# facebookresearch/vggsfm

Measured on NVIDIA H100. Metric: BA iterations/sec, higher is better.
Workload: dtype f64

## Files before the change

vggsfm_b200/csrc/chol.cu:

```cuda
#include <stdlib.h>
#include <algorithm>
#include <map>
#include <vector>
#include <tuple>
#include "common.cuh"

namespace vgg {

constexpr int CB = 128;
constexpr int CLD = 132;
constexpr int C_RPC = 16;
constexpr int C_RPC_MAX = 32;
constexpr int CT = 64;
constexpr int C_THREADS = 256;

__device__ __forceinline__ double fast_rsqrt(double p) {
  double r;
  asm("rsqrt.approx.ftz.f64 %0, %1;" : "=d"(r) : "d"(p));
  const double hp = 0.5 * p;
  r = r * fma(-hp * r, r, 1.5);
  r = r * fma(-hp * r, r, 1.5);
  return r;
}
constexpr double CHOL_PMIN = 2.2250738585072014e-308;

template <bool PROBE>
__device__ __forceinline__ int cta_chol128(double* Ls, double* dinv, int* fail_sm, int tid, int xr,
                                           long long* prof = nullptr) {
  const int lane = tid & 31, warp = tid >> 5;
  __shared__ __align__(16) double Lh[64];
  if (tid == 0) *fail_sm = 0;
  __syncthreads();
  auto tri_row = [](int e) { return (e >= 1) + (e >= 3) + (e >= 6) + (e >= 10) + (e >= 15) + (e >= 21) + (e >= 28); };
  const int pi0 = tri_row(lane), pj0 = lane - pi0 * (pi0 + 1) / 2;
  const int e1 = lane < 4 ? lane + 32 : 35;
  const int pi1 = tri_row(e1), pj1 = e1 - pi1 * (pi1 + 1) / 2;
  long long pacc[6] = {0, 0, 0, 0, 0, 0}, plast = 0;
  const bool ptid = PROBE && (tid == 0 || tid == 32);
  if (ptid) plast = clock64();
#define CHOL_MARK(ph)                         \
  if (ptid) {                                 \
    const long long t_ = clock64();           \
    pacc[ph] += t_ - plast;                   \
    plast = t_;                               \
  }
  auto leaf = [&](int c0) {
    double a[8];
    const int r = c0 + (lane & 7);
#pragma unroll
    for (int c = 0; c < 8; c += 2) {
      const double2 v = *reinterpret_cast<const double2*>(Ls + r * CLD + c0 + c);
      a[c] = v.x;
      a[c + 1] = v.y;
    }
    int fail = 0;
    double mydinv = 1.0;
#pragma unroll
    for (int j = 0; j < 8; j += 2) {
      const double A = __shfl_sync(0xffffffffu, a[j], j);
      const double B = __shfl_sync(0xffffffffu, a[j], j + 1);
      const double C = __shfl_sync(0xffffffffu, a[j + 1], j + 1);
      const double AC = A * C;
      const double det = fma(-B, B, AC);
      double ia = fast_rsqrt(A);
      double ib = (A * ia) * fast_rsqrt(det);
      double l10 = B * ia;
      const bool good = A >= CHOL_PMIN && det >= CHOL_PMIN && AC < 1e280 && AC > 1e-280;
      if (!good) {
        if (!(A >= CHOL_PMIN)) {
          if (fail == 0) fail = c0 + j + 1;
          ia = 1.0;
          l10 = B;
        }
        const double p1 = fma(-l10, l10, C);
        if (!(p1 >= CHOL_PMIN)) {
          if (fail == 0) fail = c0 + j + 2;
          ib = 1.0;
        } else {
          ib = rsqrt(p1);
        }
      }
      const double x0 = a[j] * ia;
      const double x1 = fma(-x0, l10, a[j + 1]) * ib;
      a[j] = x0;
      a[j + 1] = x1;
      if (lane == j) {
        dinv[c0 + j] = ia;
        dinv[c0 + j + 1] = ib;
        mydinv = ia;
      }
      if (lane == j + 1) mydinv = ib;
#pragma unroll
      for (int c = j + 2; c < 8; ++c) {
        const double l0 = __shfl_sync(0xffffffffu, x0, c);
        const double l1 = __shfl_sync(0xffffffffu, x1, c);
        if (lane >= c) a[c] = fma(-x1, l1, fma(-x0, l0, a[c]));
      }
    }
    if (lane < 8) {
#pragma unroll
      for (int c = 0; c < 8; ++c) Ls[r * CLD + c0 + c] = (c <= lane) ? a[c] : 0.0;
#pragma unroll
      for (int c = 0; c < 8; ++c) Lh[lane * 8 + c] = (c < lane) ? a[c] * mydinv : 0.0;
    }
    if (lane == 0 && fail && *fail_sm == 0) *fail_sm = fail;
  };
  auto row_update = [&](int r, int c0, int jb, int js, int jend) {
    double li[8];
#pragma unroll
    for (int k = 0; k < 8; k += 2) {
      const double2 v = *reinterpret_cast<const double2*>(Ls + r * CLD + c0 + k);
      li[k] = v.x;
      li[k + 1] = v.y;
    }
    int j = jb;
    for (; j + js <= jend; j += 2 * js) {
      const double* l0 = Ls + j * CLD + c0;
      const double* l1 = Ls + (j + js) * CLD + c0;
      double s0 = Ls[r * CLD + j], s1 = Ls[r * CLD + j + js];
#pragma unroll
      for (int k = 0; k < 8; k += 2) {
        const double2 u = *reinterpret_cast<const double2*>(l0 + k);
        const double2 w = *reinterpret_cast<const double2*>(l1 + k);
        s0 = fma(-li[k], u.x, s0);
        s1 = fma(-li[k], w.x, s1);
        s0 = fma(-li[k + 1], u.y, s0);
        s1 = fma(-li[k + 1], w.y, s1);
      }
      Ls[r * CLD + j] = s0;
      Ls[r * CLD + j + js] = s1;
    }
    if (j <= jend) {
      const double* l0 = Ls + j * CLD + c0;
      double s0 = Ls[r * CLD + j];
#pragma unroll
      for (int k = 0; k < 8; k += 2) {
        const double2 u = *reinterpret_cast<const double2*>(l0 + k);
        s0 = fma(-li[k], u.x, s0);
        s0 = fma(-li[k + 1], u.y, s0);
      }
      Ls[r * CLD + j] = s0;
    }
  };
  if (warp == 0) leaf(0);
  __syncthreads();
  CHOL_MARK(0)
  for (int sp = 0; sp < CB / 32; ++sp) {
    const int c32 = sp * 32;
    for (int mp = 0; mp < 4; ++mp) {
      const int c0 = c32 + mp * 8;
      {
        const int r = c0 + 8 + tid;
        if (r < CB + xr) {
          double x[8];
#pragma unroll
          for (int c = 0; c < 8; c += 2) {
            const double2 v = *reinterpret_cast<const double2*>(Ls + r * CLD + c0 + c);
            x[c] = v.x;
            x[c + 1] = v.y;
          }
#pragma unroll
          for (int m = 0; m < 8; ++m) x[m] *= dinv[c0 + m];
#pragma unroll
          for (int m = 1; m < 8; ++m) {
#pragma unroll
            for (int k = 0; k < m; ++k) x[m] = fma(-x[k], Lh[m * 8 + k], x[m]);
          }
#pragma unroll
          for (int c = 0; c < 8; c += 2) *reinterpret_cast<double2*>(Ls + r * CLD + c0 + c) = make_double2(x[c], x[c + 1]);
        }
      }
      __syncthreads();
      CHOL_MARK(1)
      if (mp < 3) {
        const int n0 = c0 + 8;
        if (warp == 0) {
          {
            const double* ri = Ls + (n0 + pi0) * CLD + c0;
            const double* rj = Ls + (n0 + pj0) * CLD + c0;
            const double* ri1 = Ls + (n0 + pi1) * CLD + c0;
            const double* rj1 = Ls + (n0 + pj1) * CLD + c0;
            double s0 = Ls[(n0 + pi0) * CLD + n0 + pj0], s1 = 0.0;
            double u0 = Ls[(n0 + pi1) * CLD + n0 + pj1], u1 = 0.0;
#pragma unroll
            for (int k = 0; k < 8; k += 4) {
              const double2 a0 = *reinterpret_cast<const double2*>(ri + k), a1 = *reinterpret_cast<const double2*>(ri + k + 2);
              const double2 b0 = *reinterpret_cast<const double2*>(rj + k), b1 = *reinterpret_cast<const double2*>(rj + k + 2);
              const double2 c0v = *reinterpret_cast<const double2*>(ri1 + k), c1v = *reinterpret_cast<const double2*>(ri1 + k + 2);
              const double2 d0 = *reinterpret_cast<const double2*>(rj1 + k), d1 = *reinterpret_cast<const double2*>(rj1 + k + 2);
              s0 = fma(-a0.x, b0.x, s0);
              s1 = fma(-a0.y, b0.y, s1);
              u0 = fma(-c0v.x, d0.x, u0);
              u1 = fma(-c0v.y, d0.y, u1);
              s0 = fma(-a1.x, b1.x, s0);
              s1 = fma(-a1.y, b1.y, s1);
              u0 = fma(-c1v.x, d1.x, u0);
              u1 = fma(-c1v.y, d1.y, u1);
            }
            Ls[(n0 + pi0) * CLD + n0 + pj0] = s0 + s1;
            if (lane < 4) Ls[(n0 + pi1) * CLD + n0 + pj1] = u0 + u1;
          }
          __syncwarp();
          leaf(n0);
        } else {
          const int t = tid - 32;
          for (int rr = t >> 1; n0 + rr < CB + xr; rr += 112) {
            const int r = n0 + rr, half = t & 1;
            const int jend = min(r, c32 + 31);
            if (r < n0 + 8) continue;
            row_update(r, c0, n0 + half, 2, jend);
          }
        }
        CHOL_MARK(2)
        __syncthreads();
        CHOL_MARK(3)
      }
    }
    const int t0 = c32 + 32;
    const int nrb = (CB - t0) / 32;
    if (nrb > 0) {
      const int ntile = nrb * (nrb + 1);
      const int nxt = xr ? (CB - t0) / 16 : 0;
      const int rend = CB + xr;
      const int g = lane >> 2, q = lane & 3;
      bool leaf_pending = warp == 0;
      for (int t = warp == 0 ? 0 : warp; t < ntile + nxt; t += (warp == 0 ? ntile + nxt : C_THREADS / 32 - 1)) {
        int R0, C0, nrow16 = 2;
        if (t < ntile) {
          int rb = 0, cb = t;
          while (cb >= 2 * rb + 2) { cb -= 2 * rb + 2; ++rb; }
          R0 = t0 + rb * 32;
          C0 = t0 + cb * 16;
        } else {
          R0 = CB;
          C0 = t0 + (t - ntile) * 16;
          nrow16 = (xr + 15) / 16;
        }
        double c[2][2][4];
#pragma unroll
        for (int i = 0; i < 2; ++i)
#pragma unroll
          for (int j = 0; j < 2; ++j) c[i][j][0] = c[i][j][1] = c[i][j][2] = c[i][j][3] = 0.0;
#pragma unroll
        for (int kk = c32; kk < c32 + 32; kk += 16) {
          double a[2][8], b[2][4];
#pragma unroll
          for (int j = 0; j < 2; ++j)
#pragma unroll
            for (int e = 0; e < 4; ++e) b[j][e] = Ls[(C0 + j * 8 + g) * CLD + kk + q + 4 * e];
#pragma unroll
          for (int i = 0; i < 2; ++i) {
            if (i < nrow16) {
#pragma unroll
              for (int e = 0; e < 8; ++e) {
                const int r = R0 + i * 16 + g + 8 * (e & 1);
                a[i][e] = r < rend ? Ls[r * CLD + kk + q + 4 * (e >> 1)] : 0.0;
              }
#pragma unroll
              for (int j = 0; j < 2; ++j) dmma_m16n8k16(c[i][j], a[i], b[j]);
            }
          }
        }
#pragma unroll
        for (int i = 0; i < 2; ++i) {
          if (i >= nrow16) continue;
#pragma unroll
          for (int h = 0; h < 2; ++h) {
            const int r = R0 + i * 16 + g + 8 * h;
            if (r >= rend) continue;
#pragma unroll
            for (int j = 0; j < 2; ++j) {
              const int col = C0 + j * 8 + 2 * q;
              if (col > r) continue;
              double* pp = Ls + r * CLD + col;
              if (col + 1 <= r) {
                double2 v = *reinterpret_cast<double2*>(pp);
                v.x -= c[i][j][2 * h];
                v.y -= c[i][j][2 * h + 1];
                *reinterpret_cast<double2*>(pp) = v;
              } else {
                *pp -= c[i][j][2 * h];
              }
            }
          }
        }
        if (leaf_pending) {
          __syncwarp();
          leaf(t0);
          leaf_pending = false;
        }
      }
      CHOL_MARK(4)
      __syncthreads();
      CHOL_MARK(5)
    }
  }
#undef CHOL_MARK
  if (ptid) {
#pragma unroll
    for (int i = 0; i < 6; ++i) prof[(tid == 32 ? 6 : 0) + i] = pacc[i];
  }
  return *fail_sm;
}

__global__ void __launch_bounds__(C_THREADS, 1) chol128_probe_kernel(const double* __restrict__ A, double* __restrict__ L,
                                                                      long long* __restrict__ prof, int reps, int xr) {
  extern __shared__ __align__(16) double cp_smem[];
  __shared__ double dinv[CB];
  __shared__ int fail_sm;
  const int tid = threadIdx.x;
  long long total = 0;
  for (int rep = 0; rep < reps; ++rep) {
    for (int e = tid; e < CB * CB; e += C_THREADS) cp_smem[(e >> 7) * CLD + (e & 127)] = A[e];
    for (int e = tid; e < xr * CB; e += C_THREADS)
      cp_smem[(CB + (e >> 7)) * CLD + (e & 127)] = A[(CB - xr + (e >> 7)) * CB + (e & 127)];
    __syncthreads();
    const long long t0 = clock64();
    cta_chol128<true>(cp_smem, dinv, &fail_sm, tid, xr, prof);
    __syncthreads();
    total = clock64() - t0;
  }
  if (tid == 0) prof[12] = total;
  for (int e = tid; e < CB * CB; e += C_THREADS) L[e] = ((e & 127) <= (e >> 7)) ? cp_smem[(e >> 7) * CLD + (e & 127)] : 0.0;
}

constexpr int CHOL_SPIN_LIMIT = 1 << 22;
constexpr int CHOL_INFO_STALLED = 0x7fffffff;

__global__ void __launch_bounds__(C_THREADS, 1) chol_panel_kernel(int n, int lda, int k0, double* __restrict__ A,
                                                                   double* __restrict__ Ldiag ,
                                                                   int* __restrict__ info, int* __restrict__ flags,
                                                                   int fuse, int band_end, int arrow_lo, int xr) {
  extern __shared__ __align__(16) double cp_smem[];
  double* Ls = cp_smem;
  double* Ts = cp_smem + CB * CLD;
  __shared__ double dinv[CB];
  __shared__ int fail_sm;
  const int tid = threadIdx.x, lane = tid & 31, warp = tid >> 5;
  const int nb = min(CB, n - k0);
  const bool solver = blockIdx.x > 0;
  const int band_hi = min(band_end, n);
  const int chunks1r = (max(0, band_hi - (k0 + CB)) + xr - 1) / xr;
  const int cidx = (int)blockIdx.x - 1;
  const int r0 = cidx < chunks1r ? k0 + CB + cidx * xr : arrow_lo + (cidx - chunks1r) * xr;
  const int nrows = solver ? min(xr, (cidx < chunks1r ? band_hi : n) - r0) : 0;
  for (int e = tid; e < CB * (CB / 2); e += C_THREADS) {
    const int i = e >> 6, j = (e & 63) * 2;
    if (i < nb) {
      cp_async16(Ls + i * CLD + j, A + (size_t)(k0 + i) * lda + k0 + j);
    } else {
      *reinterpret_cast<double2*>(Ls + i * CLD + j) = make_double2(j == i ? 1.0 : 0.0, j + 1 == i ? 1.0 : 0.0);
    }
  }
  for (int e = tid; e < xr * (CB / 2); e += C_THREADS) {
    const int r = e >> 6, j = (e & 63) * 2;
    if (r < nrows) cp_async16(Ts + r * CLD + j, A + (size_t)(r0 + r) * lda + k0 + j);
    else *reinterpret_cast<double2*>(Ts + r * CLD + j) = make_double2(0.0, 0.0);
  }
  cp_async_commit();
  cp_async_wait<0>();
  __syncthreads();
  const int fail = cta_chol128<false>(Ls, dinv, &fail_sm, tid, xr);
  if (fail && blockIdx.x == 0 && tid == 0) atomicCAS(info, 0, k0 + fail);
  if (!solver) {
    const bool alone = gridDim.x == 1;
    double* dst = Ldiag + (size_t)(k0 / CB) * CB * CB;
    for (int e = tid; e < CB * CB; e += C_THREADS) {
      const int i = e >> 7, j = e & 127;
      if (i < nb && j < nb) {
        if (j > i) A[(size_t)(k0 + i) * lda + k0 + j] = Ls[j * CLD + i];
        else if (alone) A[(size_t)(k0 + i) * lda + k0 + j] = Ls[i * CLD + j];
        else dst[e] = Ls[i * CLD + j];
      }
    }
    if (k0 > 0) {
      const double* src = Ldiag + (size_t)(k0 / CB - 1) * CB * CB;
      double* blk = A + (size_t)(k0 - CB) * lda + (k0 - CB);
      for (int e0 = tid; e0 < CB * CB; e0 += 8 * C_THREADS) {
        double v[8];
#pragma unroll
        for (int u = 0; u < 8; ++u) {
          const int e = e0 + u * C_THREADS;
          v[u] = ((e & 127) <= (e >> 7)) ? __ldcg(src + e) : 0.0;
        }
#pragma unroll
        for (int u = 0; u < 8; ++u) {
          const int e = e0 + u * C_THREADS;
          const int i = e >> 7, j = e & 127;
          if (j <= i) blk[(size_t)i * lda + j] = v[u];
        }
      }
    }
    return;
  }
  for (int e = tid; e < nrows * CB; e += C_THREADS) {
    const int r = e >> 7, c = e & 127;
    if (c < nb) A[(size_t)(r0 + r) * lda + k0 + c] = Ts[r * CLD + c];
  }
  for (int e = tid; e < nrows * CB; e += C_THREADS) {
    const int c = e / nrows, r = e - c * nrows;
    if (c < nb) A[(size_t)(k0 + c) * lda + r0 + r] = Ts[r * CLD + c];
  }
  if (!fuse) return;

  const int t0 = k0 + CB;
  const bool p_active = band_end > t0 || arrow_lo == t0;
  const int nprod = p_active ? min((CB + xr - 1) / xr, (int)gridDim.x - 1) : 0;
  if (nprod == 0) return;
  int* flag = flags + k0 / CB;
  __threadfence();
  __syncthreads();
  if (tid == 0) {
    if ((int)blockIdx.x <= nprod) atomicAdd(flag, 1);
    int spins = 0, seen;
    do {
      asm volatile("ld.acquire.gpu.global.s32 %0, [%1];" : "=r"(seen) : "l"(flag) : "memory");
    } while (seen < nprod && ++spins < CHOL_SPIN_LIMIT);
    if (seen < nprod) atomicCAS(info, 0, CHOL_INFO_STALLED);
  }
  __syncthreads();
#pragma unroll
  for (int half = 0; half < 2; ++half) {
    for (int e = tid; e < CB * 16; e += C_THREADS) {
      const int row = e >> 4, ch = (e & 15) * 4 + half * 64;
      double* dst = Ls + row * CLD + ch;
      if (t0 + row < n) {
        const double* src = A + (size_t)(t0 + row) * lda + k0 + ch;
        cp_async16(dst, src);
        cp_async16(dst + 2, src + 2);
      } else {
        *reinterpret_cast<double2*>(dst) = make_double2(0.0, 0.0);
        *reinterpret_cast<double2*>(dst + 2) = make_double2(0.0, 0.0);
      }
    }
    cp_async_commit();
  }
  {
    const int g = lane >> 2, q = lane & 3;
    const int nrow16 = (xr + 15) / 16;
    double c[2][2][4];
#pragma unroll
    for (int i = 0; i < 2; ++i)
#pragma unroll
      for (int j = 0; j < 2; ++j) c[i][j][0] = c[i][j][1] = c[i][j][2] = c[i][j][3] = 0.0;
#pragma unroll
    for (int half = 0; half < 2; ++half) {
      if (half == 0) cp_async_wait<1>();
      else cp_async_wait<0>();
      __syncthreads();
#pragma unroll 2
      for (int kk = half * 64; kk < half * 64 + 64; kk += 16) {
        double a[2][8], b[2][4];
#pragma unroll
        for (int j = 0; j < 2; ++j)
#pragma unroll
          for (int e = 0; e < 4; ++e) b[j][e] = Ls[(warp * 16 + j * 8 + g) * CLD + kk + q + 4 * e];
#pragma unroll
        for (int i = 0; i < 2; ++i) {
          if (i < nrow16) {
#pragma unroll
            for (int e = 0; e < 8; ++e) {
              const int r = i * 16 + g + 8 * (e & 1);
              a[i][e] = r < xr ? Ts[r * CLD + kk + q + 4 * (e >> 1)] : 0.0;
            }
#pragma unroll
            for (int j = 0; j < 2; ++j) dmma_m16n8k16(c[i][j], a[i], b[j]);
          }
        }
      }
    }
#pragma unroll
    for (int i = 0; i < 2; ++i) {
#pragma unroll
      for (int h = 0; h < 2; ++h) {
        const int rr = i * 16 + g + 8 * h;
        if (i >= nrow16 || rr >= nrows) continue;
        const int r = r0 + rr;
#pragma unroll
        for (int j = 0; j < 2; ++j) {
          const int col = t0 + warp * 16 + j * 8 + 2 * q;
          double* p = A + (size_t)r * lda + col;
          if (col <= r) atomicAdd(p, -c[i][j][2 * h]);
          if (col + 1 <= r) atomicAdd(p + 1, -c[i][j][2 * h + 1]);
        }
      }
    }
  }
}

constexpr int CUD = 68;
enum { CU_ALL = 0, CU_NEXT = 1, CU_REST = 2 };
__global__ void __launch_bounds__(C_THREADS, 2) chol_update_kernel(int n, int lda, int k0, int t0, int mode,
                                                                    double* __restrict__ A, int band_end, int arrow_lo,
                                                                    int all_red) {
  extern __shared__ __align__(16) double cu_smem[];
  double* As = cu_smem;
  double* Bs = cu_smem + CT * CUD;
  int bi, bj;
  {
    const int t = blockIdx.x;
    if (mode == CU_NEXT) {
      const int T = (max(0, min(band_end, n) - t0) + 63) / 64 + (band_end >= n ? 0 : (n - arrow_lo + 63) / 64);
      if (t < T - 2) { bi = 2 + t; bj = 2; }
      else { bi = 3 + (t - (T - 2)); bj = 3; }
    } else {
      bi = (int)((sqrtf(8.0f * (float)t + 1.0f) - 1.0f) * 0.5f);
      while ((bi + 1) * (bi + 2) / 2 <= t) ++bi;
      while (bi * (bi + 1) / 2 > t) --bi;
      bj = t - bi * (bi + 1) / 2;
      const int skip = mode == CU_REST ? 4 : 0;
      bi += skip;
      bj += skip;
    }
  }
  const bool diag = bi == bj;
  const int tid = threadIdx.x, lane = tid & 31, warp = tid >> 5;
  const int T1v = band_end >= n ? (1 << 30) : (band_end - t0) / 64;
  auto vrow = [&](int v) { return v < T1v ? t0 + v * 64 : arrow_lo + (v - T1v) * 64; };
  const int ri = vrow(bi), rj = vrow(bj);
  const double* bs = diag ? As : Bs;
  const int wm = warp / 4, wn = warp % 4;
  const int g = lane >> 2, q = lane & 3;
  double c[2][2][4];
#pragma unroll
  for (int i = 0; i < 2; ++i)
#pragma unroll
    for (int j = 0; j < 2; ++j) c[i][j][0] = c[i][j][1] = c[i][j][2] = c[i][j][3] = 0.0;
  const double* arow = As + (wm * 32 + g) * CUD + q;
  const double* brow = bs + (wn * 16 + g) * CUD + q;
#pragma unroll 1
  for (int half = 0; half < 2; ++half) {
    if (half) __syncthreads();
    for (int e = tid; e < 2 * CT * 16; e += C_THREADS) {
      const int row = e >> 4, ch = (e & 15) * 4;
      const bool isA = row < CT;
      if (!isA && diag) continue;
      const int grow = isA ? ri + row : rj + (row - CT);
      double* dst = (isA ? As + row * CUD : Bs + (row - CT) * CUD) + ch;
      if (grow < n) {
        const double* src = A + (size_t)grow * lda + k0 + half * 64 + ch;
        cp_async16(dst, src);
        cp_async16(dst + 2, src + 2);
      } else {
        *reinterpret_cast<double2*>(dst) = make_double2(0.0, 0.0);
        *reinterpret_cast<double2*>(dst + 2) = make_double2(0.0, 0.0);
      }
    }
    cp_async_commit();
    cp_async_wait<0>();
    __syncthreads();
#pragma unroll 2
    for (int kk = 0; kk < 64; kk += 16) {
      double a[2][8], b[2][4];
#pragma unroll
      for (int i = 0; i < 2; ++i)
#pragma unroll
        for (int e = 0; e < 8; ++e) a[i][e] = arow[(i * 16 + 8 * (e & 1)) * CUD + kk + 4 * (e >> 1)];
#pragma unroll
      for (int j = 0; j < 2; ++j)
#pragma unroll
        for (int e = 0; e < 4; ++e) b[j][e] = brow[j * 8 * CUD + kk + 4 * e];
#pragma unroll
      for (int i = 0; i < 2; ++i)
#pragma unroll
        for (int j = 0; j < 2; ++j) dmma_m16n8k16(c[i][j], a[i], b[j]);
    }
  }
  const bool red = all_red || mode == CU_NEXT || (mode == CU_REST && bj < 6);
#pragma unroll
  for (int i = 0; i < 2; ++i) {
#pragma unroll
    for (int h = 0; h < 2; ++h) {
      const int r = ri + wm * 32 + i * 16 + g + 8 * h;
      if (r >= n) continue;
#pragma unroll
      for (int j = 0; j < 2; ++j) {
        const int col = rj + wn * 16 + j * 8 + 2 * q;
        if (col > r) continue;
        double* p = A + (size_t)r * lda + col;
        const double v0 = c[i][j][2 * h], v1 = c[i][j][2 * h + 1];
        if (red) {
          atomicAdd(p, -v0);
          if (col + 1 <= r) atomicAdd(p + 1, -v1);
        } else if (col + 1 <= r) {
          double2 v = *reinterpret_cast<double2*>(p);
          v.x -= v0;
          v.y -= v1;
          *reinterpret_cast<double2*>(p) = v;
        } else {
          *p -= v0;
        }
      }
    }
  }
}


size_t chol_workspace_doubles(int n) {
  const int nblk = (n + CB - 1) / CB;
  return (size_t)nblk * CB * CB + (size_t)(nblk + 1) / 2 + 1;
}

namespace {

struct CholStreams {
  cudaStream_t side_lo = nullptr, side_mid = nullptr, cap = nullptr;
  cudaEvent_t ev_col = nullptr, ev_upd[2] = {nullptr, nullptr}, ev_bulk[3] = {nullptr, nullptr, nullptr};
  bool ready = false;
};

int chol_streams(CholStreams** out) {
  static thread_local CholStreams s;
  if (!s.ready) {
    int lo = 0, hi = 0;
    VGG_CUDA_CHECK(cudaDeviceGetStreamPriorityRange(&lo, &hi));
    VGG_CUDA_CHECK(cudaStreamCreateWithPriority(&s.side_lo, cudaStreamNonBlocking, lo));
    VGG_CUDA_CHECK(cudaStreamCreateWithPriority(&s.side_mid, cudaStreamNonBlocking, (lo + hi) / 2));
    VGG_CUDA_CHECK(cudaStreamCreateWithPriority(&s.cap, cudaStreamNonBlocking, hi));
    VGG_CUDA_CHECK(cudaEventCreateWithFlags(&s.ev_col, cudaEventDisableTiming));
    VGG_CUDA_CHECK(cudaEventCreateWithFlags(&s.ev_upd[0], cudaEventDisableTiming));
    VGG_CUDA_CHECK(cudaEventCreateWithFlags(&s.ev_upd[1], cudaEventDisableTiming));
    for (int i = 0; i < 3; ++i) VGG_CUDA_CHECK(cudaEventCreateWithFlags(&s.ev_bulk[i], cudaEventDisableTiming));
    s.ready = true;
  }
  *out = &s;
  return VGG_OK;
}

int chol_sms() {
  static const int v = [] {
    int dev = 0, sms = 0;
    if (cudaGetDevice(&dev) != cudaSuccess || cudaDeviceGetAttribute(&sms, cudaDevAttrMultiProcessorCount, dev) != cudaSuccess)
      sms = 0;
    return sms > 0 ? sms : 132;
  }();
  return v;
}

int chol_set_attrs() {
  static bool done = false;
  if (done) return VGG_OK;
  VGG_CUDA_CHECK(cudaFuncSetAttribute(chol_panel_kernel, cudaFuncAttributeMaxDynamicSharedMemorySize,
                                      (int)(sizeof(double) * (CB + C_RPC_MAX) * CLD)));
  VGG_CUDA_CHECK(cudaFuncSetAttribute(chol_update_kernel, cudaFuncAttributeMaxDynamicSharedMemorySize,
                                      (int)(sizeof(double) * 2 * CT * CUD)));
  done = true;
  return VGG_OK;
}

}

std::vector<int> g_chol_band_end;
int g_chol_arrow_blk = 0;

namespace {

int chol_panel_rows(int below1, int below2, int* chunks) {
  const int sms = chol_sms();
  int xr = C_RPC;
  for (;; xr += 4) {
    *chunks = (below1 + xr - 1) / xr + (below2 + xr - 1) / xr;
    if (1 + *chunks <= sms || xr >= C_RPC_MAX) return xr;
  }
}

int chol_enqueue(int n, int lda, double* A, double* Ldiag, int* info, int* flags, cudaStream_t st, CholStreams* cs,
                 bool lookahead) {
  const int nblk = (n + CB - 1) / CB;
  const size_t smem_u = sizeof(double) * 2 * CT * CUD;
  const bool banded = lookahead && (int)g_chol_band_end.size() >= nblk && g_chol_arrow_blk > 0;
  auto band_rows = [&](int b, int* band_end, int* arrow_lo) {
    if (!banded) {
      *band_end = *arrow_lo = n;
      return;
    }
    *band_end = std::min(n, g_chol_band_end[b] * CB);
    *arrow_lo = std::min(n, std::max(g_chol_arrow_blk * CB, *band_end));
    if (*band_end >= n || *arrow_lo <= *band_end) *band_end = *arrow_lo = n;
  };
  auto panel = [&](int b) -> int {
    const int k0 = b * CB;
    int band_end, arrow_lo, chunks;
    band_rows(b, &band_end, &arrow_lo);
    const int below1 = std::max(0, std::min(band_end, n) - (k0 + CB));
    const int below2 = band_end >= n ? 0 : n - arrow_lo;
    const int xr = chol_panel_rows(below1, below2, &chunks);
    const size_t smem_p = sizeof(double) * (CB + xr) * CLD;
    const int fuse = lookahead ? 1 : 0;
    chol_panel_kernel<<<1 + chunks, C_THREADS, smem_p, st>>>(n, lda, k0, A, Ldiag, info, flags, fuse, band_end, arrow_lo, xr);
    VGG_LAUNCH_CHECK();
    return VGG_OK;
  };
  int rc;
  if ((rc = panel(0))) return rc;
  if (!lookahead) {
    for (int b = 0; b + 1 < nblk; ++b) {
      const int k0 = b * CB, t0 = k0 + CB;
      const int T = (n - t0 + CT - 1) / CT;
      chol_update_kernel<<<T * (T + 1) / 2, C_THREADS, smem_u, st>>>(n, lda, k0, t0, CU_ALL, A, n, n, 0);
      VGG_LAUNCH_CHECK();
      if ((rc = panel(b + 1))) return rc;
    }
    return VGG_OK;
  }
  bool have_u1[2] = {false, false}, have_u2[3] = {false, false, false};
  for (int b = 0; b + 1 < nblk; ++b) {
    const int k0 = b * CB, t0 = k0 + CB;
    int band_end, arrow_lo;
    band_rows(b, &band_end, &arrow_lo);
    const int T = (std::max(0, std::min(band_end, n) - t0) + CT - 1) / CT + (band_end >= n ? 0 : (n - arrow_lo + CT - 1) / CT);
    const int all_red = band_end >= n ? 0 : 1;
    const int n_u1 = T > 2 ? (T - 2) + (T > 3 ? T - 3 : 0) : 0;
    const int n_u2 = T > 4 ? (T - 4) * (T - 3) / 2 : 0;
    have_u1[b & 1] = false;
    have_u2[b % 3] = false;
    if (n_u1 > 0) {
      VGG_CUDA_CHECK(cudaEventRecord(cs->ev_col, st));
      VGG_CUDA_CHECK(cudaStreamWaitEvent(cs->side_mid, cs->ev_col, 0));
      if (b >= 2 && have_u2[(b - 2) % 3]) VGG_CUDA_CHECK(cudaStreamWaitEvent(cs->side_mid, cs->ev_bulk[(b - 2) % 3], 0));
      chol_update_kernel<<<n_u1, C_THREADS, smem_u, cs->side_mid>>>(n, lda, k0, t0, CU_NEXT, A, band_end, arrow_lo, all_red);
      VGG_LAUNCH_CHECK();
      VGG_CUDA_CHECK(cudaEventRecord(cs->ev_upd[b & 1], cs->side_mid));
      have_u1[b & 1] = true;
      if (n_u2 > 0) {
        VGG_CUDA_CHECK(cudaStreamWaitEvent(cs->side_lo, cs->ev_col, 0));
        chol_update_kernel<<<n_u2, C_THREADS, smem_u, cs->side_lo>>>(n, lda, k0, t0, CU_REST, A, band_end, arrow_lo, all_red);
        VGG_LAUNCH_CHECK();
        VGG_CUDA_CHECK(cudaEventRecord(cs->ev_bulk[b % 3], cs->side_lo));
        have_u2[b % 3] = true;
      }
    }
    if (b >= 1 && have_u1[(b - 1) & 1]) VGG_CUDA_CHECK(cudaStreamWaitEvent(st, cs->ev_upd[(b - 1) & 1], 0));
    if (b >= 2 && have_u2[(b - 2) % 3]) VGG_CUDA_CHECK(cudaStreamWaitEvent(st, cs->ev_bulk[(b - 2) % 3], 0));
    if ((rc = panel(b + 1))) return rc;
  }
  for (int i = 0; i < 2; ++i)
    if (have_u1[i]) VGG_CUDA_CHECK(cudaStreamWaitEvent(st, cs->ev_upd[i], 0));
  for (int i = 0; i < 3; ++i)
    if (have_u2[i]) VGG_CUDA_CHECK(cudaStreamWaitEvent(st, cs->ev_bulk[i], 0));
  return VGG_OK;
}

}

int chol_lower_inplace(int n, int lda, double* A, double* Ldiag, int* info, cudaStream_t st) {
  VGG_REQUIRE((lda % 2) == 0, "lda must be even");
  int rc;
  if ((rc = chol_set_attrs())) return rc;
  VGG_CUDA_CHECK(cudaMemsetAsync(info, 0, sizeof(int), st));
  const int nblk0 = (n + CB - 1) / CB;
  int* flags = reinterpret_cast<int*>(Ldiag + (size_t)nblk0 * CB * CB);
  VGG_CUDA_CHECK(cudaMemsetAsync(flags, 0, sizeof(int) * (size_t)nblk0, st));
  static const bool use_graph = [] { const char* e = getenv("VGG_CHOL_GRAPH"); return !(e && e[0] == '0'); }();
  const int nblk = (n + CB - 1) / CB;
  CholStreams* cs = nullptr;
  if ((rc = chol_streams(&cs))) return rc;
  if (nblk < 3 || !use_graph) return chol_enqueue(n, lda, A, Ldiag, info, flags, st, cs, nblk >= 3);
  typedef std::tuple<double*, int, int, int*, double*, unsigned long long> Key;
  static thread_local std::map<Key, cudaGraphExec_t> cache;
  unsigned long long band_hash = (unsigned long long)g_chol_arrow_blk;
  for (int v : g_chol_band_end) band_hash = band_hash * 1000003ull + (unsigned long long)(v + 1);
  const Key key(A, n, lda, info, Ldiag, band_hash);
  auto it = cache.find(key);
  if (it == cache.end()) {
    const long long launches_before = g_launch_count;
    cudaGraph_t graph = nullptr;
    VGG_CUDA_CHECK(cudaStreamBeginCapture(cs->cap, cudaStreamCaptureModeThreadLocal));
    rc = chol_enqueue(n, lda, A, Ldiag, info, flags, cs->cap, cs, true);
    const cudaError_t ce = cudaStreamEndCapture(cs->cap, &graph);
    g_launch_count = launches_before;
    if (rc) {
      if (graph) cudaGraphDestroy(graph);
      return rc;
    }
    VGG_CUDA_CHECK(ce);
    cudaGraphExec_t exec = nullptr;
    VGG_CUDA_CHECK(cudaGraphInstantiate(&exec, graph, 0));
    cudaGraphDestroy(graph);
    if (cache.size() > 8) {
      for (auto& kv : cache) cudaGraphExecDestroy(kv.second);
      cache.clear();
    }
    it = cache.emplace(key, exec).first;
  }
  VGG_CUDA_CHECK(cudaGraphLaunch(it->second, st));
  g_launch_count += 1 + 3 * (nblk - 1);
  return VGG_OK;
}

}

extern "C" int vgg_dev_chol128_probe(int reps, const double* A_host, double* L_host, long long* prof13_host) {
  using namespace vgg;
  VGG_REQUIRE(A_host && L_host && prof13_host && reps > 0, "chol128 probe: bad arguments");
  double *dA = nullptr, *dL = nullptr;
  long long* dP = nullptr;
  VGG_CUDA_CHECK(cudaMalloc(&dA, sizeof(double) * CB * CB));
  VGG_CUDA_CHECK(cudaMalloc(&dL, sizeof(double) * CB * CB));
  VGG_CUDA_CHECK(cudaMalloc(&dP, sizeof(long long) * 13));
  VGG_CUDA_CHECK(cudaMemcpy(dA, A_host, sizeof(double) * CB * CB, cudaMemcpyHostToDevice));
  VGG_CUDA_CHECK(cudaMemset(dP, 0, sizeof(long long) * 13));
  const int smem = (int)(sizeof(double) * (CB + C_RPC) * CLD);
  VGG_CUDA_CHECK(cudaFuncSetAttribute(chol128_probe_kernel, cudaFuncAttributeMaxDynamicSharedMemorySize, smem));
  chol128_probe_kernel<<<1, C_THREADS, smem>>>(dA, dL, dP, reps, C_RPC);
  VGG_LAUNCH_CHECK();
  VGG_CUDA_CHECK(cudaDeviceSynchronize());
  VGG_CUDA_CHECK(cudaMemcpy(L_host, dL, sizeof(double) * CB * CB, cudaMemcpyDeviceToHost));
  VGG_CUDA_CHECK(cudaMemcpy(prof13_host, dP, sizeof(long long) * 13, cudaMemcpyDeviceToHost));
  cudaFree(dA);
  cudaFree(dL);
  cudaFree(dP);
  return VGG_OK;
}

extern "C" int vgg_dev_set_chol_band(const int* end_blk_host, int count, int arrow_blk) {
  using namespace vgg;
  g_chol_band_end.assign(end_blk_host, end_blk_host + (count > 0 ? count : 0));
  g_chol_arrow_blk = count > 0 ? arrow_blk : 0;
  return VGG_OK;
}
```

Baseline: 346.8.

## Precompute leaf pivot shuffles and honor stream priorities in captured Cholesky graph

The 8x8 leaf factorization now gathers all 2x2 pivot entries up front and updates them locally from the already-shuffled L values, which takes shuffles off the serial dependency chain. The captured Cholesky graph's kernel nodes are given explicit priorities (panel high, next-update mid, bulk update low), and the graph is instantiated with the node-priority flag so the critical-path panel kernels are favored during replay. The leaf update also drops the lane predicate and updates every lane unconditionally, which may change the values held in the upper triangle. The node lookup relies on matching kernel function pointers and reading the kernel parameter at index 4.

```diff
diff --git a/vggsfm_b200/csrc/chol.cu b/vggsfm_b200/csrc/chol.cu
--- a/vggsfm_b200/csrc/chol.cu
+++ b/vggsfm_b200/csrc/chol.cu
@@ -53,13 +53,20 @@
       a[c] = v.x;
       a[c + 1] = v.y;
     }
+    double pa[4], pb[4], pc[4];
+#pragma unroll
+    for (int q = 0; q < 4; ++q) {
+      pa[q] = __shfl_sync(0xffffffffu, a[2 * q], 2 * q);
+      pb[q] = __shfl_sync(0xffffffffu, a[2 * q], 2 * q + 1);
+      pc[q] = __shfl_sync(0xffffffffu, a[2 * q + 1], 2 * q + 1);
+    }
     int fail = 0;
     double mydinv = 1.0;
 #pragma unroll
     for (int j = 0; j < 8; j += 2) {
-      const double A = __shfl_sync(0xffffffffu, a[j], j);
-      const double B = __shfl_sync(0xffffffffu, a[j], j + 1);
-      const double C = __shfl_sync(0xffffffffu, a[j + 1], j + 1);
+      const double A = pa[j / 2];
+      const double B = pb[j / 2];
+      const double C = pc[j / 2];
       const double AC = A * C;
       const double det = fma(-B, B, AC);
       double ia = fast_rsqrt(A);
@@ -90,11 +97,18 @@
         mydinv = ia;
       }
       if (lane == j + 1) mydinv = ib;
+      double l0[8], l1[8];
 #pragma unroll
       for (int c = j + 2; c < 8; ++c) {
-        const double l0 = __shfl_sync(0xffffffffu, x0, c);
-        const double l1 = __shfl_sync(0xffffffffu, x1, c);
-        if (lane >= c) a[c] = fma(-x1, l1, fma(-x0, l0, a[c]));
+        l0[c] = __shfl_sync(0xffffffffu, x0, c);
+        l1[c] = __shfl_sync(0xffffffffu, x1, c);
+        a[c] = fma(-x1, l1[c], fma(-x0, l0[c], a[c]));
+      }
+#pragma unroll
+      for (int q = j / 2 + 1; q < 4; ++q) {
+        pa[q] = fma(-l1[2 * q], l1[2 * q], fma(-l0[2 * q], l0[2 * q], pa[q]));
+        pb[q] = fma(-l1[2 * q + 1], l1[2 * q], fma(-l0[2 * q + 1], l0[2 * q], pb[q]));
+        pc[q] = fma(-l1[2 * q + 1], l1[2 * q + 1], fma(-l0[2 * q + 1], l0[2 * q + 1], pc[q]));
       }
     }
     if (lane < 8) {
@@ -606,6 +620,7 @@
 struct CholStreams {
   cudaStream_t side_lo = nullptr, side_mid = nullptr, cap = nullptr;
   cudaEvent_t ev_col = nullptr, ev_upd[2] = {nullptr, nullptr}, ev_bulk[3] = {nullptr, nullptr, nullptr};
+  int prio_lo = 0, prio_mid = 0, prio_hi = 0;
   bool ready = false;
 };
 
@@ -614,8 +629,11 @@
   if (!s.ready) {
     int lo = 0, hi = 0;
     VGG_CUDA_CHECK(cudaDeviceGetStreamPriorityRange(&lo, &hi));
+    s.prio_lo = lo;
+    s.prio_mid = (lo + hi) / 2;
+    s.prio_hi = hi;
     VGG_CUDA_CHECK(cudaStreamCreateWithPriority(&s.side_lo, cudaStreamNonBlocking, lo));
-    VGG_CUDA_CHECK(cudaStreamCreateWithPriority(&s.side_mid, cudaStreamNonBlocking, (lo + hi) / 2));
+    VGG_CUDA_CHECK(cudaStreamCreateWithPriority(&s.side_mid, cudaStreamNonBlocking, s.prio_mid));
     VGG_CUDA_CHECK(cudaStreamCreateWithPriority(&s.cap, cudaStreamNonBlocking, hi));
     VGG_CUDA_CHECK(cudaEventCreateWithFlags(&s.ev_col, cudaEventDisableTiming));
     VGG_CUDA_CHECK(cudaEventCreateWithFlags(&s.ev_upd[0], cudaEventDisableTiming));
@@ -738,6 +756,38 @@
     if (have_u1[i]) VGG_CUDA_CHECK(cudaStreamWaitEvent(st, cs->ev_upd[i], 0));
   for (int i = 0; i < 3; ++i)
     if (have_u2[i]) VGG_CUDA_CHECK(cudaStreamWaitEvent(st, cs->ev_bulk[i], 0));
+  return VGG_OK;
+}
+
+int chol_set_node_priorities(cudaGraph_t graph, const CholStreams* cs, int npanels) {
+  size_t nn = 0;
+  VGG_CUDA_CHECK(cudaGraphGetNodes(graph, nullptr, &nn));
+  std::vector<cudaGraphNode_t> nodes(nn);
+  VGG_CUDA_CHECK(cudaGraphGetNodes(graph, nodes.data(), &nn));
+  int panels = 0;
+  for (cudaGraphNode_t node : nodes) {
+    cudaGraphNodeType type;
+    VGG_CUDA_CHECK(cudaGraphNodeGetType(node, &type));
+    if (type != cudaGraphNodeTypeKernel) continue;
+    cudaKernelNodeParams kp;
+    VGG_CUDA_CHECK(cudaGraphKernelNodeGetParams(node, &kp));
+    int want;
+    if (kp.func == reinterpret_cast<void*>(chol_panel_kernel)) {
+      want = cs->prio_hi;
+      ++panels;
+    } else if (kp.func == reinterpret_cast<void*>(chol_update_kernel)) {
+      want = *static_cast<const int*>(kp.kernelParams[4]) == CU_NEXT ? cs->prio_mid : cs->prio_lo;
+    } else {
+      continue;
+    }
+    cudaLaunchAttributeValue v;
+    VGG_CUDA_CHECK(cudaGraphKernelNodeGetAttribute(node, cudaLaunchAttributePriority, &v));
+    if (v.priority != want) {
+      v.priority = want;
+      VGG_CUDA_CHECK(cudaGraphKernelNodeSetAttribute(node, cudaLaunchAttributePriority, &v));
+    }
+  }
+  VGG_REQUIRE(panels == npanels, "captured Cholesky graph: panel kernel nodes not found");
   return VGG_OK;
 }
 
@@ -774,8 +824,12 @@
       return rc;
     }
     VGG_CUDA_CHECK(ce);
+    if ((rc = chol_set_node_priorities(graph, cs, nblk))) {
+      cudaGraphDestroy(graph);
+      return rc;
+    }
     cudaGraphExec_t exec = nullptr;
-    VGG_CUDA_CHECK(cudaGraphInstantiate(&exec, graph, 0));
+    VGG_CUDA_CHECK(cudaGraphInstantiate(&exec, graph, cudaGraphInstantiateFlagUseNodePriority));
     cudaGraphDestroy(graph);
     if (cache.size() > 8) {
       for (auto& kv : cache) cudaGraphExecDestroy(kv.second);
```

New measurement: 354.3, median of 6. 2.2% higher.
